# simensov/ml4ca

Hardware: AMD Instinct MI355X
Metric: env-steps/sec at 65536 parallel envs (higher is better)
Workload: dtype f32

## Files before the change

include/dpenv.h:

```cpp
#ifndef DPENV_H
#define DPENV_H

#include <stddef.h>
#include <stdint.h>

#ifdef __cplusplus
extern "C" {
#endif

#define DPENV_ABI_VERSION 6

typedef struct dpenv_s* dpenv_handle;
typedef void* dpenv_stream;

enum {
    DPENV_OK = 0,
    DPENV_EINVAL = -1,
    DPENV_ENODEV = -2,
    DPENV_ENOMEM = -3,
    DPENV_EHIP = -4,
};

enum { DPENV_FULL = 0, DPENV_SIMPLE = 1, DPENV_LIMITED = 2, DPENV_FINAL = 3 };
enum { DPENV_AOS = 0 , DPENV_SOA = 1  };
// ... 80 lines not shown
const char* dpenv_last_error(dpenv_handle h);

int dpenv_set_reset_fraction(dpenv_handle h, float fraction);
int dpenv_set_vessel_class(dpenv_handle h, const int32_t* class_id, dpenv_stream s);

enum { DPENV_VESSEL_KEEP_RANDOMISATION = 1 };
int dpenv_set_vessel_params_ex(dpenv_handle h, const float* params, uint32_t flags, dpenv_stream s);
int dpenv_set_vessel_params(dpenv_handle h, const float* params, dpenv_stream s);
int dpenv_get_vessel_params(dpenv_handle h, float* params_out, dpenv_stream s);
int dpenv_set_vessel_randomisation(dpenv_handle h, const float* nominal, const float* rel_range, dpenv_stream s);
int dpenv_set_current(dpenv_handle h, const float* vc, const float* beta, dpenv_stream s);
int dpenv_set_current_present(dpenv_handle h, const float* vc, const float* beta, dpenv_stream s);
int dpenv_get_current(dpenv_handle h, float* vc_out, float* beta_out, dpenv_stream s);
int dpenv_get_current_mean(dpenv_handle h, float* vc_out, float* beta_out, dpenv_stream s);
int dpenv_set_current_randomisation(dpenv_handle h, const float* vc_nominal, const float* beta_nominal, float vc_range, float beta_range,
                                    dpenv_stream s);

int dpenv_reset(dpenv_handle h, const uint8_t* mask, const float* init, const float* ref, void* obs_out,
                dpenv_stream s);

int dpenv_step(dpenv_handle h, const float* action, const float* new_ref, void* obs_out, float* rew_out,
               uint8_t* done_out, dpenv_stream s);
int dpenv_step_ex(dpenv_handle h, const dpenv_step_io* io, dpenv_stream s);

#define DPENV_MAX_SWITCH 8
typedef struct dpenv_rollout_io {
    uint32_t struct_size;
    int32_t T;
    const float* actions;
    void* obs;
    float* reward;
    uint8_t* done;
    int32_t n_switch;
    int32_t switch_step[DPENV_MAX_SWITCH];
    const float* refs;
} dpenv_rollout_io;
int dpenv_rollout(dpenv_handle h, const dpenv_rollout_io* io, dpenv_stream s);

enum { DPENV_ACT_LEAKY_RELU = 0, DPENV_ACT_TANH = 1 };
typedef struct dpenv_mlp {
    int32_t n_layers;
    int32_t sizes[6];
    const float* W[5];
    const float* b[5];
} dpenv_mlp;
enum { DPENV_POLICY_F16 = 0, DPENV_POLICY_F32 = 1, DPENV_POLICY_F32_ACTOR = 2 };
// ... 204 lines not shown
```

ml4ca_amd/_lib.py:

```python
import ctypes as C
import os

_HERE = os.path.dirname(os.path.abspath(__file__))
LIB_PATH = os.environ.get('DPENV_LIB') or os.path.join(_HERE, 'lib', 'libdpenv.so')

OK, EINVAL, ENODEV, ENOMEM, EHIP = 0, -1, -2, -3, -4
FULL, SIMPLE, LIMITED, FINAL = 0, 1, 2, 3
AOS, SOA = 0, 1
WRAP_REFERENCE, WRAP_RADIANS = 0, 1
F32, BF16 = 0, 1
ACT_LEAKY_RELU, ACT_TANH = 0, 1
IMITATE_NLL, IMITATE_MSE = 0, 1
POLICY_F16, POLICY_F32, POLICY_F32_ACTOR = 0, 1, 2
LAUNCH_AUTO, LAUNCH_ONE_WAVE, LAUNCH_TWO_WAVE = 0, 1, 2
DONE_TERMINAL, DONE_TIMELIMIT, DONE_FAULT = 1, 2, 4
NSTATE, NPARAM, NPARAM_USED, MAX_CLASSES = 15, 32, 32, 64
ABI_VERSION = 6
VESSEL_KEEP_RANDOMISATION = 1

S = dict(N=0, E=1, PSI=2, U=3, V=4, R=5, REF_N=6, REF_E=7, REF_PSI=8,
         PT_BOW=9, PT_PORT=10, PT_STAR=11, A_BOW=12, A_PORT=13, A_STAR=14)
P = dict(M11=0, M22=1, M23=2, M33=3, XU=4, XUU=5, YV=6, YVV=7, YR=8, NV=9, NR=10, NRR=11,
         KF_BOW=12, KF_PORT=13, KF_STAR=14, KR_BOW=15, KR_PORT=16, KR_STAR=17,
         LX_BOW=18, LX_PORT=19, LX_STAR=20, LY_BOW=21, LY_PORT=22, LY_STAR=23, NUV=24, YUR=25,
# ... 87 lines not shown
    'dpenv_abi_version': (C.c_int, []),
    'dpenv_default_config': (C.c_int, [C.POINTER(Config)]),
    'dpenv_default_vessel': (C.c_int, [C.POINTER(C.c_float)]),
    'dpenv_default_vessel_ex': (C.c_int, [C.c_int32, C.POINTER(C.c_float)]),
    'dpenv_act_dim': (C.c_int, [C.POINTER(Config)]),
    'dpenv_obs_dim': (C.c_int, [C.POINTER(Config)]),
    'dpenv_create': (C.c_int, [C.POINTER(Config), C.POINTER(C.c_float), _I32, C.POINTER(_VP)]),
    'dpenv_destroy': (C.c_int, [_VP]),
    'dpenv_last_error': (C.c_char_p, [_VP]),
    'dpenv_set_reset_fraction': (C.c_int, [_VP, _F]),
    'dpenv_set_vessel_class': (C.c_int, [_VP, _VP, _VP]),
    'dpenv_set_vessel_params': (C.c_int, [_VP, _VP, _VP]),
    'dpenv_set_vessel_params_ex': (C.c_int, [_VP, _VP, C.c_uint32, _VP]),
    'dpenv_get_vessel_params': (C.c_int, [_VP, _VP, _VP]),
    'dpenv_set_vessel_randomisation': (C.c_int, [_VP, C.POINTER(C.c_float), C.POINTER(C.c_float), _VP]),
    'dpenv_set_current': (C.c_int, [_VP, _VP, _VP, _VP]),
    'dpenv_set_current_present': (C.c_int, [_VP, _VP, _VP, _VP]),
    'dpenv_get_current': (C.c_int, [_VP, _VP, _VP, _VP]),
    'dpenv_get_current_mean': (C.c_int, [_VP, _VP, _VP, _VP]),
    'dpenv_set_current_randomisation': (C.c_int, [_VP, _VP, _VP, _F, _F, _VP]),
    'dpenv_reset': (C.c_int, [_VP, _VP, _VP, _VP, _VP, _VP]),
    'dpenv_step': (C.c_int, [_VP, _VP, _VP, _VP, _VP, _VP, _VP]),
    'dpenv_step_ex': (C.c_int, [_VP, C.POINTER(StepIO), _VP]),
    'dpenv_rollout': (C.c_int, [_VP, C.POINTER(RolloutIO), _VP]),
    'dpenv_set_policy': (C.c_int, [_VP, C.POINTER(Mlp), C.POINTER(Mlp), C.POINTER(C.c_float), _F]),
    'dpenv_set_policy_ex': (C.c_int, [_VP, C.POINTER(Mlp), C.POINTER(Mlp), C.POINTER(C.c_float), C.c_int32, _F]),
    'dpenv_set_policy_desc': (C.c_int, [_VP, C.POINTER(PolicyDesc), _VP]),
    'dpenv_policy_forward': (C.c_int, [_VP, _VP, _VP, _VP, _I32, _VP]),
    'dpenv_policy_rollout': (C.c_int, [_VP, C.POINTER(PolicyRolloutIO), _VP]),
    'dpenv_get_state': (C.c_int, [_VP, _VP, _VP, _VP]),
    'dpenv_set_state': (C.c_int, [_VP, _VP, _VP, _VP]),
    'dpenv_get_rng_counters': (C.c_int, [_VP, _VP, _VP, _VP]),
    'dpenv_set_rng_counters': (C.c_int, [_VP, _VP, _VP, _VP]),
    'dpenv_get_obs_thrust': (C.c_int, [_VP, _VP, _VP]),
    'dpenv_get_policy_launch': (C.c_int, [_VP, C.POINTER(C.c_int32), C.POINTER(C.c_int32)]),
    'dpenv_get_policy_launch_ex': (C.c_int, [_VP, C.POINTER(C.c_int32)]),
    'dpenv_release_policy_graphs': (C.c_int, [_VP]),
    'dpenv_set_obs_thrust': (C.c_int, [_VP, _VP, _VP]),
    'dpenv_thrust_map': (C.c_int, [C.POINTER(C.c_float), _VP, _VP, _VP, _I32, _VP]),
    'dpenv_gae': (C.c_int, [_VP, _VP, _VP, _VP, _VP, _I32, _I32, _F, _F, _VP, _VP, _VP]),
    'dpenv_gae_workspace_bytes': (C.c_int64, [_I32]),
    'dpenv_gae_stats': (C.c_int, [_VP, _VP, _VP, _VP, _VP, _I32, _I32, _F, _F, _VP, _VP, _VP, _VP, _VP]),
    'dpenv_adv_apply_stats': (C.c_int, [_VP, _I64, _VP, C.c_double, _VP]),
    'dpenv_adv_sum': (C.c_int, [_VP, _I64, _VP, _VP]),
    'dpenv_adv_sumsq': (C.c_int, [_VP, _I64, _VP, _VP, _VP]),
    'dpenv_adv_apply': (C.c_int, [_VP, _I64, _VP, _VP, _VP]),
# ... 78 lines not shown
```

ml4ca_amd/csrc/dpenv_api.hip:

```cpp
#include <cmath>
#include <cstdarg>
#include <cstdio>
#include <cstring>
#include <memory>
#include <new>
#include <string>

#include "dpenv_host.h"

using namespace dpenv;
using namespace dpenv::host;

enum { LOSS_OFF = 0, LOSS_ON = 1, LOSS_UNKNOWN = 2 };

#pragma GCC visibility push(hidden)
struct dpenv_s {
    dpenv_config cfg = {};
    StepArgs args = {};
    int mode = 0;
    int n_classes = 1;
    float* blob = nullptr;
    size_t blob_bytes = 0;
    float* cur_vc = nullptr;
    float* cur_beta = nullptr;
// ... 527 lines not shown
    DeviceGuard dev_guard(h->device);
    if (!io || io->struct_size != sizeof(dpenv_step_io)) return fail(h, DPENV_EINVAL, "dpenv_step_io ABI mismatch");
    if (h->integ_on) return fail(h, DPENV_EINVAL, INTEG_OPEN_LOOP_MSG, "dpenv_step");
    if (h->reff_on) return fail(h, DPENV_EINVAL, REFF_OPEN_LOOP_MSG, "dpenv_step");
    if (!io->action || !io->obs || !io->reward || !io->done)
        return fail(h, DPENV_EINVAL, "action, obs, reward and done buffers are required");
    if (int rc = require_classes(h)) return rc;
    StepArgs a = h->args;
    bind_optional(h, a, (hipStream_t)s);
    a.action = io->action;
    a.new_ref = io->new_ref;
    a.obs = io->obs;
    a.rew = io->reward;
    a.done = io->done;
    a.parts = io->reward_parts;
    a.final_obs = io->final_obs;
    if (!h->has_policy) a.S3 = nullptr;
    const int reset_wave = (!h->cfg.step_one_wave && (int64_t)h->cfg.n_envs <= (int64_t)256 * h->n_cus) ? 1 : 0;
    HIP_TRY(h, dev::launch_step(&a, h->mode, h->cfg.extended_state, vessel_source(h), reset_wave, (hipStream_t)s));
    h->lag_valid = h->has_policy;
    return DPENV_OK;
}

extern "C" int dpenv_step(dpenv_handle h, const float* action, const float* new_ref, void* obs_out, float* rew_out,
                          uint8_t* done_out, dpenv_stream s)
{
    dpenv_step_io io = {};
    io.struct_size = (uint32_t)sizeof io;
    io.action = action; io.new_ref = new_ref; io.obs = obs_out; io.reward = rew_out; io.done = done_out;
    return dpenv_step_ex(h, &io, s);
}

extern "C" int dpenv_rollout(dpenv_handle h, const dpenv_rollout_io* io, dpenv_stream s)
{
    if (!h) return DPENV_EINVAL;
    DeviceGuard dev_guard(h->device);
    if (!io || io->struct_size != sizeof(dpenv_rollout_io)) return fail(h, DPENV_EINVAL, "dpenv_rollout_io ABI mismatch");
    if (h->integ_on) return fail(h, DPENV_EINVAL, INTEG_OPEN_LOOP_MSG, "dpenv_rollout");
    if (h->reff_on) return fail(h, DPENV_EINVAL, REFF_OPEN_LOOP_MSG, "dpenv_rollout");
    if (io->T <= 0 || !io->actions || !io->obs || !io->reward || !io->done)
        return fail(h, DPENV_EINVAL, "T > 0 and action, obs, reward, done blocks are required");
    if (int rc = check_schedule(h, io)) return rc;
    if (int rc = require_classes(h)) return rc;
    StepArgs a = h->args;
    bind_optional(h, a, (hipStream_t)s);
    RolloutArgs ra = {};
// ... 602 lines not shown
```

ml4ca_amd/csrc/dpenv_dev.h:

```cpp
#ifndef DPENV_DEV_H
#define DPENV_DEV_H

#include <hip/hip_runtime.h>
#include <stdint.h>
#include <type_traits>

namespace dpenv {

constexpr int BLOCK = 64;
constexpr int RBLOCK = 64;
constexpr int MAX_SWITCH = 8;
constexpr int CTRL_NPARAM = 32, CTRL_KP = 0, CTRL_KD = 3, CTRL_KI = 6, CTRL_ZB = 9, CTRL_TMAX = 12, CTRL_WEIGHT = 15, CTRL_LX = 20,
              CTRL_LY = 23, CTRL_KF = 26, CTRL_KR_BOW = 29, CTRL_F_EPS = 30;
constexpr int CTRL_TAB_STREAMS = 9;
constexpr int64_t ctrl_tab_float4s(int n) { return ((int64_t)n + 63) / 64 * 64 * CTRL_TAB_STREAMS; }
constexpr int MAX_CLASSES = 64;

enum { MODE_FULL = 0, MODE_SIMPLE = 1, MODE_LIMITED = 2, MODE_FINAL_WRAP = 3, MODE_FINAL_CONT = 4 };
enum { LAYOUT_AOS = 0, LAYOUT_SOA = 1 };
enum { WRAP_REFERENCE = 0, WRAP_RADIANS = 1 };
enum { DONE_TERMINAL = 1u, DONE_TIMELIMIT = 2u, DONE_FAULT = 4u };

enum {
    VD_M11 = 0, VD_M22, VD_M23, VD_INV11, VD_I22, VD_I23, VD_I33,
// ... 283 lines not shown
struct ScoreArgs {
    uint4* state;
    const void* obs;
    const float* act;
    const float* rew;
    const uint8_t* done;
    const float* integ;
    int T, n, obs_stride, act_stride, cut_at_end;
    float dt;
    float norm[3], coeff[3], rps[3];
};

struct LabelArgs {
    const void* obs;
    const uint8_t* done;
    const float* z_in;
    float* z_out;
    float* act;
    int T, n;
};

namespace __attribute__((visibility("hidden"))) dev {
hipError_t launch_step(const StepArgs* a, int mode, int ext, int ves, int reset_wave, hipStream_t s);
hipError_t launch_rollout(const StepArgs* a, const RolloutArgs* ra, int mode, int ext, int ves, int two_wave, hipStream_t s);
hipError_t launch_reset(const StepArgs* a, int mode, int ext, const uint8_t* mask, const float* init, const float* ref, hipStream_t s);
hipError_t launch_get_state(const StepArgs* a, float* st, int32_t* ctr, hipStream_t s);
hipError_t launch_set_state(const StepArgs* a, const float* st, const int32_t* ctr, hipStream_t s);
hipError_t launch_pack_env_vessels(const float* raw, int64_t p_stride, int64_t i_stride, float4* tab, uint32_t* loss_flag, int stride, int n,
                                   hipStream_t s);
hipError_t launch_unpack_env_vessels(const float4* tab, int stride, float* out, int n, hipStream_t s);
hipError_t launch_thrust_map(const VesselDev* vd, const float* n_pct, const float* alpha, float* tau, int n, hipStream_t s);
int64_t gae_workspace_bytes(int n);
hipError_t launch_gae(const float* rew, const float* val, const uint8_t* end, const float* boot, const float* last_val, int T, int n,
                      float gamma, float lam, float* adv, float* ret, double* workspace, double* stats, hipStream_t s);
int64_t score_state_bytes(int n);
int64_t score_summary_workspace_bytes(int n);
hipError_t launch_score(const ScoreArgs* a, int obs_bf16, hipStream_t s);
hipError_t launch_score_read(const void* state, int n, double* out, hipStream_t s);
hipError_t launch_score_summary(const void* state, int n, double* out, double* workspace, hipStream_t s);
hipError_t launch_sum(const float* x, int64_t count, const float* mean, float* out, hipStream_t s);
hipError_t launch_adv_apply(float* x, int64_t count, const float* mean, const float* std, const double* stats, double total_count,
                            hipStream_t s);
hipError_t launch_pack_policy(const PackNet* pi, const PackNet* v, const float* log_std, int adim, int ks, int nent, int nblk, int split,
                              void* frags, float* bias, float* consts, hipStream_t s);
hipError_t launch_policy_forward(const PolicyArgs* pa, int od, int adim, const float* obs, float* mu, float* v, int n, hipStream_t s);
hipError_t launch_policy_forward_x(const PolicyArgs* pa, int od, int adim, const float* obs, float* mu, float* v, int n, hipStream_t s);
// ... 22 lines not shown
```

ml4ca_amd/csrc/dpenv_env_dev.h:

```cpp
#ifndef DPENV_ENV_DEV_H
#define DPENV_ENV_DEV_H
#include <hip/hip_runtime.h>
#include <hip/hip_bf16.h>
#include <stdint.h>

#include "dpenv_dev.h"

namespace dpenv {

constexpr float kPi = 3.14159265358979323846f;

__device__ __forceinline__ void philox4x32_10(uint32_t c0, uint32_t c1, uint32_t c2, uint32_t c3, uint32_t k0,
                                              uint32_t k1, uint32_t out[4])
{
#pragma unroll
    for (int r = 0; r < 10; ++r) {
        const uint64_t p0 = (uint64_t)c0 * 0xD2511F53ull, p1 = (uint64_t)c2 * 0xCD9E8D57ull;
        const uint32_t hi0 = (uint32_t)(p0 >> 32), lo0 = (uint32_t)p0, hi1 = (uint32_t)(p1 >> 32), lo1 = (uint32_t)p1;
        const uint32_t n0 = hi1 ^ c1 ^ k0, n2 = hi0 ^ c3 ^ k1;
        c0 = n0; c1 = lo1; c2 = n2; c3 = lo0;
        k0 += 0x9E3779B9u; k1 += 0xBB67AE85u;
    }
    out[0] = c0; out[1] = c1; out[2] = c2; out[3] = c3;
}
// ... 589 lines not shown
        ang[1] = clipf(w3 * kPi, kPi); ang[2] = clipf(w4 * kPi, kPi);
    } else if (MODE == MODE_FINAL_CONT) {
        if (!DEFER_ANG) { ang[1] = clipf(atan2_lean(act[3], act[4]), kPi); ang[2] = clipf(atan2_lean(act[5], act[6]), kPi); }
    }
}

template <int MODE, bool DEFER_ANG = false>
__device__ __forceinline__ void env_decode(const Vessel& ve, float ang[3], const float* act, Wrench& w, const ThrustLoss* tl = nullptr)
{
    env_decode_cmd<MODE, DEFER_ANG>(ang, act, w.thr);
    if (MODE == MODE_FINAL_CONT) {
        float sc[4];
        const float np2 = fmaf(act[3], act[3], act[4] * act[4]), ns2 = fmaf(act[5], act[5], act[6] * act[6]);
        const float ip = __builtin_amdgcn_rsqf(np2), is = __builtin_amdgcn_rsqf(ns2);
        constexpr float kMinNormal = 1.17549435e-38f;
        sc[0] = (np2 >= kMinNormal) ? act[3] * ip : 0.0f; sc[1] = (np2 >= kMinNormal) ? act[4] * ip : copysignf(1.0f, act[4]);
        sc[2] = (ns2 >= kMinNormal) ? act[5] * is : 0.0f; sc[3] = (ns2 >= kMinNormal) ? act[6] * is : copysignf(1.0f, act[6]);
        thrust_map(ve, w.thr, ang, w.tx, w.ty, w.tn, sc, tl);
    } else {
        thrust_map(ve, w.thr, ang, w.tx, w.ty, w.tn, nullptr, tl);
    }
}

__device__ __forceinline__ void env_plant(const StepArgs& a, const Vessel& ve, float tx, float ty, float tn, bool cur, float vcN,
                                          float vcE, float& N, float& E, float& psi, float& u, float& v, float& r, float sn, float cs)
{
    if (cur) {
        u -= fmaf(cs, vcN, sn * vcE);
        v -= fmaf(cs, vcE, -(sn * vcN));
    }
    const float h = a.h;
    const float hA = h * ve.inv11, h22 = h * ve.i22, h23 = h * ve.i23, h33 = h * ve.i33;
    const float yur = ve.Yur + ve.m11;
    const float nuv = ve.Nuv - ve.m11;
    const int nsub = a.hold_plant ? 0 : a.n_substeps;
    float aN = 0.0f, aE = 0.0f;
#pragma unroll 10
    for (int k = 0; k < nsub; ++k) {
        const float q = fmaf(ve.m22, v, ve.m23 * r);
        float fx = fmaf(-fmaf(ve.Xuu, fabsf(u), ve.Xu), u, tx);
        fx = fmaf(q, r, fx);
        float fy = fmaf(-fmaf(ve.Yvv, fabsf(v), ve.Yv), v, ty);
        fy = fmaf(-fmaf(yur, u, ve.Yr), r, fy);
        float fn = fmaf(-q, u, tn);
        fn = fmaf(-fmaf(nuv, u, ve.Nv), v, fn);
        fn = fmaf(-fmaf(ve.Nrr, fabsf(r), ve.Nr), r, fn);
        u = fmaf(hA, fx, u);
        v = fmaf(h22, fy, fmaf(h23, fn, v));
        r = fmaf(h23, fy, fmaf(h33, fn, r));
        aN = fmaf(-sn, v, fmaf(cs, u, aN));
        aE = fmaf(cs, v, fmaf(sn, u, aE));
        const float d = h * r;
        const float e = -0.5f * d;
        psi += d;
        const float c2 = fmaf(fmaf(e, cs, -sn), d, cs);
        const float s2n = fmaf(fmaf(e, sn, cs), d, sn);
        cs = c2; sn = s2n;
// ... 54 lines not shown
        for (int k = 0; k < 6; ++k) t = t || (fabsf(o[k]) > b[k]);
        d = t ? DONE_TERMINAL : 0u;
    }
    {
        float chk = s.N + s.E + s.psi + s.u + s.v + s.r;
#pragma unroll
        for (int k = 0; k < ModeTraits<MODE>::A; ++k) chk += act[k];
        if (!(fabsf(chk) <= 3.0e38f)) d |= DONE_TERMINAL | DONE_FAULT;
    }
    if (has_ref) { s.refN = nrN; s.refE = nrE; s.refPsi = nrP; }
    s.steps += 1;
    if (a.max_ep_len > 0 && s.steps >= a.max_ep_len) d |= DONE_TIMELIMIT;
    s.pt[0] = thr[0]; s.pt[1] = thr[1]; s.pt[2] = thr[2];
    out.d = d;
}

struct StepRest {
    float thr[3], pt_old[3], ang_prev[3], ang_new[3];
};

template <int MODE, bool EXT, bool DEFER>
__device__ __forceinline__ void env_step_chain(const StepArgs& a, const Vessel& ve, Env& s, const float* act, bool has_ref,
                                               float nrN, float nrE, float nrP, bool cur, float vcN, float vcE, StepOut& out, StepRest& rest,
                                               int il = -1)
{
#pragma unroll
    for (int k = 0; k < 3; ++k) { rest.ang_prev[k] = s.ang[k]; rest.pt_old[k] = s.pt[k]; }
    Wrench w;
    if (il == IL_SHARED || (il >= 0 && thrust_loss_on(a))) {
        ThrustLoss tl;
        if (il == IL_SHARED) {
#pragma unroll
            for (int k = 0; k < 3; ++k) { tl.klf[k] = a.kl[k]; tl.klr[k] = a.kl[3 + k]; }
        } else {
            const float4 q0 = a.env_tab[(int64_t)ENV_GROUPS * a.env_stride + il], q1 = a.env_tab[(int64_t)(ENV_GROUPS + 1) * a.env_stride + il];
            tl.klf[0] = q0.x; tl.klf[1] = q0.y; tl.klf[2] = q0.z; tl.klr[0] = q0.w; tl.klr[1] = q1.x; tl.klr[2] = q1.y;
        }
        tl.u = s.u; tl.v = s.v; tl.r = s.r;
        if (cur) {
            tl.u -= fmaf(s.cs, vcN, s.sn * vcE);
            tl.v -= fmaf(s.cs, vcE, -(s.sn * vcN));
        }
        env_decode<MODE, DEFER>(ve, s.ang, act, w, &tl);
    } else {
        env_decode<MODE, DEFER>(ve, s.ang, act, w);
    }
#pragma unroll
    for (int k = 0; k < 3; ++k) { rest.thr[k] = w.thr[k]; rest.ang_new[k] = s.ang[k]; }
    float N = s.N, E = s.E, psi = s.psi, u = s.u, v = s.v, r = s.r;
    env_plant(a, ve, w.tx, w.ty, w.tn, cur, vcN, vcE, N, E, psi, u, v, r, s.sn, s.cs);
    const bool deg = (a.wrap_mode == WRAP_REFERENCE);
    float* o = out.o;
    bool same;
    float se, ce;
    {
        make_obs(N, E, psi, 0.0f, 0.0f, 0.0f, s.refN, s.refE, s.refPsi, rest.pt_old, deg, o, se, ce, same);
        if (!same) sincos_lean(psi, se, ce);
    }
    env_plant_finish(cur, vcN, vcE, se, ce, u, v);
    o[3] = u; o[4] = v; o[5] = r;
    s.N = N; s.E = E; s.psi = psi; s.u = u; s.v = v; s.r = r;
    s.sn = se; s.cs = ce;
    env_done<MODE>(a, s, act, o, rest.thr, has_ref, nrN, nrE, nrP, out);
}

template <int MODE, bool EXT, bool DEFER>
__device__ __forceinline__ void env_step_finish(const StepArgs& a, Env& s, const float* act, StepRest& rest, bool untouched, StepOut& out)
{
    if (DEFER && MODE == MODE_FINAL_CONT) {
        rest.ang_new[1] = clipf(atan2_lean(act[3], act[4]), kPi);
        rest.ang_new[2] = clipf(atan2_lean(act[5], act[6]), kPi);
        if (untouched) { s.ang[1] = rest.ang_new[1]; s.ang[2] = rest.ang_new[2]; }
    }
// ... 96 lines not shown
```

ml4ca_amd/csrc/dpenv_kernels.hip:

```cpp
#include "dpenv_env_dev.h"

namespace dpenv {

constexpr int RESETW_FIELDS = 18;
constexpr int RESETW_FIELDS_RND = 20;

template <int MODE>
__device__ __forceinline__ void reset_wave(const StepArgs& a, float* lds, int lane, int blk)
{
    const int n = a.n;
    const int i = blk * 64 + lane;
    const int il = i < n ? i : n - 1;
    const uint32_t ep = (uint32_t)a.episode[il];
    const float4 rf = a.RF[il];
    Env s;
    s.refN = rf.x; s.refE = rf.y; s.refPsi = rf.z;
    if (a.new_ref) { s.refN = a.new_ref[il]; s.refE = a.new_ref[(int64_t)n + il]; s.refPsi = a.new_ref[2 * (int64_t)n + il]; }
    ResetDraw d;
    reset_draw<MODE>(a, a.env_id_base + i, ep, d);
    float o[9];
    reset_apply<MODE>(a, s, d, o);
    lds[0 * 64 + lane] = s.N; lds[1 * 64 + lane] = s.E; lds[2 * 64 + lane] = s.psi;
#pragma unroll
    for (int k = 0; k < 9; ++k) lds[(3 + k) * 64 + lane] = o[k];
// ... 70 lines not shown
    lds_order<BLOCK>();
    const __amdgpu_buffer_rsrc_t rObs = buf_rsrc(a.obs, n * (4u * OD));
#pragma unroll
    for (int j = 0; j < OD; ++j) buf_store1(rObs, oobs + j * (4u * BLOCK), lds_io[j * BLOCK + tid]);
    __builtin_amdgcn_sched_barrier(0);
    env_step_finish<MODE, EXT, false>(a, s, act, rest, true, out);
    buf_store1(buf_rsrc(a.rew, n * 4u), o4, out.reward);
}

struct BufDesc {
    const void* base;
    uint32_t bytes;
    uint32_t flags;
};
constexpr uint32_t BUF_FLAGS = 0x00020000;
struct StepFixedArgs {
    VesselDev v0;
    float h, inv_dt;
    int32_t pad;
    BufDesc obs, done, rew, new_ref;
    int32_t terminate, max_ep_len;
};
static_assert(sizeof(StepFixedArgs) == 200 && offsetof(StepFixedArgs, obs) == 128, "StepFixedArgs layout");
constexpr int STEP_FIXED_SUBSTEPS = 20;

__device__ __forceinline__ __amdgpu_buffer_rsrc_t buf_rsrc(const BufDesc& d)
{
    __builtin_assume((reinterpret_cast<uintptr_t>(d.base) >> 48) == 0);
    return __builtin_amdgcn_make_buffer_rsrc(const_cast<void*>(d.base), 0, (int)d.bytes, (int)d.flags);
}
template <typename T> __device__ __forceinline__ void fetch_sgpr(T& x) { asm volatile("" : "+s"(x)); }
__device__ __forceinline__ void fetch_sgpr(BufDesc& d) { fetch_sgpr(d.base); fetch_sgpr(d.bytes); fetch_sgpr(d.flags); }

template <int MODE, bool EXT, bool DEG, bool ENDS, bool REF>
__global__ __launch_bounds__(BLOCK) void step_fixed_kernel(float4* S0, float4* S1, float4* S2, float4* RF, const float* action, int n_,
                                                           const StepFixedArgs fx_)
{
    constexpr int A = ModeTraits<MODE>::A;
    constexpr int OD = EXT ? 9 : 6;
    __shared__ float lds_io[BLOCK * 9];
    const int tid = threadIdx.x;
    const uint32_t n = (uint32_t)n_;
    const uint32_t i = blockIdx.x * BLOCK + tid;
    const uint32_t o16 = i * 16u, o4 = i * 4u;
    const uint32_t oact = (blockIdx.x * (BLOCK * A) + tid) * 4u;
    const uint32_t oobs = (blockIdx.x * (BLOCK * OD) + tid) * 4u;
    const __amdgpu_buffer_rsrc_t rS0 = buf_rsrc(S0, n * 16u), rS1 = buf_rsrc(S1, n * 16u), rS2 = buf_rsrc(S2, n * 16u),
                                 rRF = buf_rsrc(RF, n * 16u), rAct = buf_rsrc(action, n * (4u * A));
    StepFixedArgs fx = fx_;
    StepArgs a;
    a.h = fx.h; a.inv_dt = fx.inv_dt;
    a.n_substeps = STEP_FIXED_SUBSTEPS; a.hold_plant = 0;
    a.wrap_mode = DEG ? WRAP_REFERENCE : WRAP_RADIANS;

    float act[A];
#pragma unroll
// ... 22 lines not shown
#pragma unroll
    for (int j = 0; j < A; ++j) lds_io[j * BLOCK + tid] = act[j];
    lds_order<BLOCK>();
#pragma unroll
    for (int k = 0; k < A; ++k) act[k] = lds_io[tid * A + k];
    const Vessel ve = vessel_from_args(fx.v0);

    StepOut out;
    StepRest rest;
    env_step_chain<MODE, EXT, false>(a, ve, s, act, REF, nrN, nrE, nrP, false, 0.0f, 0.0f, out, rest, IL_NONE);
    buf_store4(rS0, o16, s.N, s.E, s.psi, s.u);
    buf_store4(rS1, o16, s.v, s.r, s.ang[1], s.ang[2]);
    buf_store4(rS2, o16, s.pt[0], s.pt[1], s.pt[2], __int_as_float(s.steps));
    if (REF || MODE == MODE_FULL) buf_store4(rRF, o16, s.refN, s.refE, s.refPsi, s.ang[0]);
    buf_store_u8(buf_rsrc(fx.done), i, (uint8_t)out.d);
    __builtin_amdgcn_sched_barrier(0);
    lds_order<BLOCK>();
#pragma unroll
    for (int k = 0; k < OD; ++k) lds_io[tid * OD + k] = out.o[k];
    lds_order<BLOCK>();
    const __amdgpu_buffer_rsrc_t rObs = buf_rsrc(fx.obs);
#pragma unroll
    for (int j = 0; j < OD; ++j) buf_store1(rObs, oobs + j * (4u * BLOCK), lds_io[j * BLOCK + tid]);
    __builtin_amdgcn_sched_barrier(0);
    env_step_finish<MODE, EXT, false>(a, s, act, rest, true, out);
    buf_store1(buf_rsrc(fx.rew), o4, out.reward);
}

template <int MODE, bool EXT, int VES, bool RESETW = false, bool LEAN = false>
__global__ __launch_bounds__(RESETW ? 2 * BLOCK : BLOCK) void step_kernel(const StepArgs a)
{
    const float4 *pS0 = a.S0, *pS1 = a.S1, *pS2 = a.S2, *pRF = a.RF;
    const float* paction = a.action;
    const int pn = a.n, playout = a.action_layout;
    constexpr int A = ModeTraits<MODE>::A;
    constexpr int OD = EXT ? 9 : 6;
    constexpr bool PER_CLASS = VES == VES_CLASS_LDS;
    constexpr bool RND = VES == VES_ENV_RND;
    constexpr bool ENV_VGPR = VES == VES_ENV_VGPR || RND;
    constexpr int IL = VES == VES_ARGS_LOSS ? IL_SHARED : IL_NONE;
    constexpr bool CURR = RND || VES == VES_ARGS_LOSS;
    __shared__ float lds_io[BLOCK * 9];
    __shared__ float lds_cls[PER_CLASS ? VD_COUNT * MAX_CLASSES : 1];
    __shared__ float4 lds_pe[VES == VES_ENV_LDS ? ENV_GROUPS * 64 : 1];
    __shared__ float lds_rst[RESETW ? (CURR ? RESETW_FIELDS_RND : RESETW_FIELDS) * 64 : 1];
    __shared__ uint32_t lds_fin[RESETW ? 64 : 1];
// ... 883 lines not shown

#include "dpenv_score_dev.h"

}

using namespace dpenv;

static bool vessel_source_ok(const StepArgs& a, int ves)
{
    return !(ves >= VES_ENV_VGPR && ves <= VES_ENV_RND && !a.env_tab) && (ves == VES_ARGS_LOSS) == (a.loss_on == LOSS_SHARED);
}

static bool step_lean_ok(const StepArgs& a, int ves)
{
    return ves == VES_ARGS && !a.auto_reset && !a.final_obs && !a.parts && !a.cur_vc && !a.current_drift && !a.S3 && !a.obs_bf16 &&
           a.obs_layout == LAYOUT_AOS && a.action_layout == LAYOUT_AOS && (int64_t)a.n * 36 < ((int64_t)1 << 31);
}

template <typename F> static hipError_t with_flag(bool on, F&& f)
{
    return on ? f(std::true_type{}) : f(std::false_type{});
}

hipError_t dev::launch_step(const StepArgs* a, int mode, int ext, int ves, int reset_wave, hipStream_t s)
{
    if (!vessel_source_ok(*a, ves)) return hipErrorInvalidValue;
    const dim3 grid((a->n + BLOCK - 1) / BLOCK);
    const bool two = a->auto_reset && reset_wave;
    const bool lean = step_lean_ok(*a, ves);
    return with_mode_ext(mode, ext, [&](auto M, auto E) {
        if (lean && a->n_substeps == STEP_FIXED_SUBSTEPS && !a->hold_plant) {
            StepFixedArgs fx;
            fx.v0 = a->v0;
            fx.h = a->h; fx.inv_dt = a->inv_dt; fx.pad = 0;
            const uint32_t n = (uint32_t)a->n;
            constexpr uint32_t OD = decltype(E)::value ? 9u : 6u;
            fx.obs = {a->obs, n * (4u * OD), BUF_FLAGS};
            fx.done = {a->done, n, BUF_FLAGS};
            fx.rew = {a->rew, n * 4u, BUF_FLAGS};
            fx.new_ref = {a->new_ref, n * 12u, BUF_FLAGS};
            fx.terminate = a->terminate; fx.max_ep_len = a->max_ep_len;
            return with_flag(a->wrap_mode == WRAP_REFERENCE, [&](auto DEG) {
                return with_flag(a->terminate || a->max_ep_len > 0, [&](auto ENDS) { return with_flag(a->new_ref != nullptr, [&](auto REF) {
                    hipLaunchKernelGGL((step_fixed_kernel<M, E, DEG, ENDS, REF>), grid, dim3(BLOCK), 0, s, a->S0, a->S1, a->S2, a->RF, a->action,
                                       a->n, fx);
                    return hipGetLastError();
                }); });
            });
        }
        if (lean) {
            hipLaunchKernelGGL((step_kernel<M, E, VES_ARGS, false, true>), grid, dim3(BLOCK), 0, s, *a);
            return hipGetLastError();
        }
        return with_ves(ves, [&](auto V) {
            if (two) hipLaunchKernelGGL((step_kernel<M, E, V, true>), grid, dim3(2 * BLOCK), 0, s, *a);
            else hipLaunchKernelGGL((step_kernel<M, E, V>), grid, dim3(BLOCK), 0, s, *a);
            return hipGetLastError();
        });
    });
}

hipError_t dev::launch_pack_env_vessels(const float* raw, int64_t p_stride, int64_t i_stride, float4* tab, uint32_t* loss_flag, int stride, int n,
                                        hipStream_t s)
{
    hipLaunchKernelGGL(pack_env_vessels_kernel, dim3((n + BLOCK - 1) / BLOCK), dim3(BLOCK), 0, s, raw, p_stride, i_stride, tab, loss_flag, stride, n);
    return hipGetLastError();
}

hipError_t dev::launch_unpack_env_vessels(const float4* tab, int stride, float* out, int n, hipStream_t s)
{
    hipLaunchKernelGGL(unpack_env_vessels_kernel, dim3((n + BLOCK - 1) / BLOCK), dim3(BLOCK), 0, s, tab, stride, out, n);
    return hipGetLastError();
}
// ... 115 lines not shown
```

ml4ca_amd/env.py:

```python
import ctypes as C
import math
import weakref

import numpy as np

from . import _lib
from .deploy import REFERENCE_FILTER_OMEGA, REFERENCE_FILTER_ZETA
from . import reset_samplers as simtools

_VARIANTS = {'full': _lib.FULL, 'simple': _lib.SIMPLE, 'limited': _lib.LIMITED, 'final': _lib.FINAL}
_NAMES = {'full': 'full', 'simple': 'revoltsimple', 'limited': 'revoltlimited', 'final': 'revoltfinal'}


def variant_constants(variant, cont_ang=False):
    pi = math.pi
    if variant == 'full':
        return dict(num_actions=6, real_action_bounds=[100] * 3 + [pi] * 3,
                    real_ss_bounds=[8.0, 8.0, pi / 2, 1.4, 0.30, 0.52],
                    default_actions={0: 0, 1: 0, 2: 0, 3: 0, 4: 0, 5: 0},
                    valid_action_indices=[0, 1, 2, 3, 4, 5],
                    act_2_act_map={0: 0, 1: 1, 2: 2, 3: 3, 4: 4, 5: 5},
                    act_2_act_map_inv={0: 0, 1: 1, 2: 2, 3: 3, 4: 4, 5: 5})
    if variant == 'simple':
        return dict(num_actions=3, real_action_bounds=[100] * 3,
# ... 14 lines not shown


class Box(object):

    def __init__(self, low, high, dtype=np.float64):
        self.low, self.high, self.shape, self.dtype = low, high, low.shape, dtype

    def sample(self):
        return np.random.uniform(self.low, self.high).astype(self.dtype)


def _torch():
    import torch
    return torch


class BatchedRevoltEnv(object):

    def __init__(self, n_envs, variant='final', extended_state=True, cont_ang=True, device='cuda:0',
                 testing=False, realtime=False, max_ep_len=800, auto_reset=False, terminate=True,
                 wrap_mode='reference', seed=0, env_id_base=0, obs_dtype='float32', current=False,
                 vessel_params=None, layout='aos', reset_fraction=0.8, time_limit=True, hold_plant=False,
                 current_drift=False, current_tau=100.0, current_sigma_v=0.02, current_sigma_beta=5.0 * math.pi / 180.0,
                 n_steps=None, reset_acts=False, step_one_wave=False, per_env_lds=False):
        torch = _torch()
        if not torch.cuda.is_available():
            raise RuntimeError('BatchedRevoltEnv needs a ROCm device: the env.step path is a HIP kernel and has no CPU fallback')
        self.lib = _lib.load()
        self.device = torch.device(device)
        self.variant = variant
        k = variant_constants(variant, cont_ang)
        self.name = _NAMES[variant]
        self.extended_state = bool(extended_state)
        self.cont_ang = bool(cont_ang) and variant == 'final'
        self.testing = bool(testing)
        self.reset_actions = bool(reset_acts)
        self.n_envs = int(n_envs)
        self.num_actions = k['num_actions']
        self.num_states = 9 if extended_state else 6
        self.real_action_bounds = k['real_action_bounds']
        self.real_ss_bounds = k['real_ss_bounds']
        self.default_actions = k['default_actions']
        self.valid_action_indices = k['valid_action_indices']
        self.act_2_act_map = k['act_2_act_map']
        self.act_2_act_map_inv = k['act_2_act_map_inv']
        self.n_steps = 1 if (testing and realtime) else 20
        if n_steps is not None:
            self.n_steps = int(n_steps)
        self.dt = 0.01 * self.n_steps
        self.max_ep_len = int(max_ep_len * 10.0 / self.n_steps)
        self.vel_rew_coeffs = [0.5, 0.5, 1.0]
        self.covar = np.array([[1.0, 0.0], [0.0, 25.0]])
        self.observation_space = Box(-np.ones(self.num_states), np.ones(self.num_states))
        self.action_space = Box(-np.ones(self.num_actions), np.ones(self.num_actions))

        cfg = _lib.default_config()
        cfg.n_envs = self.n_envs
        cfg.device = self.device.index if self.device.index is not None else torch.cuda.current_device()
        cfg.variant = _VARIANTS[variant]
        cfg.extended_state = int(self.extended_state)
        cfg.cont_ang = int(self.cont_ang)
        cfg.n_substeps = self.n_steps
        cfg.substep_dt = 0.01
        cfg.wrap_mode = {'reference': _lib.WRAP_REFERENCE, 'radians': _lib.WRAP_RADIANS}[wrap_mode]
        cfg.terminate = int(bool(terminate))
        cfg.max_ep_len = self.max_ep_len if time_limit else 0
        cfg.auto_reset = int(bool(auto_reset))
        lay = {'aos': _lib.AOS, 'soa': _lib.SOA}[layout]
        cfg.action_layout = lay
        cfg.obs_layout = lay
        self.obs_torch_dtype = {'float32': torch.float32, 'bfloat16': torch.bfloat16}[str(obs_dtype).replace('torch.', '')]
        cfg.obs_dtype = _lib.BF16 if self.obs_torch_dtype == torch.bfloat16 else _lib.F32
        cfg.current_enabled = int(bool(current))
        cfg.seed = int(seed)
        cfg.env_id_base = int(env_id_base)
        cfg.reset_fraction = float(reset_fraction)
        cfg.hold_plant = int(bool(hold_plant))
        cfg.current_drift = int(bool(current_drift))
        cfg.current_tau = float(current_tau)
        cfg.current_sigma_v = float(current_sigma_v)
        cfg.current_sigma_beta = float(current_sigma_beta)
        cfg.reset_acts = int(self.reset_actions)
        cfg.step_one_wave = int(bool(step_one_wave))
        cfg.per_env_lds = int(bool(per_env_lds))
        self.cfg = cfg
        self.layout = layout
# ... 100 lines not shown
        f32, chk = self._f32, self._chk
        chk(action, self._ashape, f32, 'action')
        if out is None:
            obs, rew, done = self._next_obs(), self._rew, self._done
        else:
            obs, rew, done = out
            chk(obs, self._oshape, self.obs_torch_dtype, 'out[0]')
            chk(rew, self._n1, f32, 'out[1]')
            chk(done, self._n1, self._u8, 'out[2]')
        io = self._io
        io.action = action.data_ptr()
        io.new_ref = chk(new_ref, self._r3, f32, 'new_ref').data_ptr() if new_ref is not None else None
        io.obs = obs.data_ptr()
        io.reward = rew.data_ptr()
        io.done = done.data_ptr()
        io.reward_parts = chk(reward_parts, self._p4, f32, 'reward_parts').data_ptr() if reward_parts is not None else None
        io.final_obs = chk(final_obs, self._oshape, self.obs_torch_dtype, 'final_obs').data_ptr() if final_obs is not None else None
        rc = self._step_ex(self._h, self._io_ref, self._stream())
        if rc:
            self._refuse_open_loop('step')
            _lib.check(rc, self._h)
        return obs, rew, done, {'None': 0}

    def _refuse_open_loop(self, what):
        if self.integral_action is not None:
            raise ValueError('%s(): the integral action is on (set_integral_action) and this launch\'s observations would lack I; fly the closed '
                             'loop (policy.policy_rollout), compose step() with deploy.BatchedBodyFrameIntegrator after set_integral_action(None), '
                             'or turn it off' % what)
        if self.reference_filter is not None:
            raise ValueError('%s(): the reference filter is on (set_reference_filter) and would not see this launch; fly the closed loop '
                             '(policy.policy_rollout), compose step() with deploy.BatchedReferenceFilter (its position as new_ref) after '
                             'set_reference_filter(None), or turn it off' % what)

    def rollout(self, actions, switch_steps=(), refs=None, out=None):
        torch = _torch()
        self._refuse_open_loop('rollout')
        T = int(actions.shape[0])
        n = self.n_envs
        self._chk(actions, (T,) + self.action_shape, torch.float32, 'actions')
        k = len(switch_steps)
        if k > 8:
            raise ValueError('at most 8 setpoint switches per rollout launch')
        if k:
            self._chk(refs, (k, 3, n), torch.float32, 'refs')
        if out is None:
            obs = torch.empty((T,) + self.obs_shape, dtype=self.obs_torch_dtype, device=self.device)
# ... 461 lines not shown
```

Measured before the change: 14.79 billion.

## Add wide fixed-step kernel with vectorized block-staged action/obs I/O

Adds a step_fixed_wide_kernel used when n is a multiple of 4 and the action/obs pointers are 16-byte aligned. It loads actions and stores observations as per-block float4 rows staged through LDS, instead of per-element strided scalar accesses. It also precomputes the plant constants on the host and passes them as kernel arguments, avoiding per-thread recomputation. The kernel argument block grows, and the new path adds extra LDS barriers plus more code to maintain. It also exposes a dpenv_step_form query and a substep_dt option.

```diff
diff --git a/include/dpenv.h b/include/dpenv.h
--- a/include/dpenv.h
+++ b/include/dpenv.h
@@ -126,6 +126,8 @@
 int dpenv_step(dpenv_handle h, const float* action, const float* new_ref, void* obs_out, float* rew_out,
                uint8_t* done_out, dpenv_stream s);
 int dpenv_step_ex(dpenv_handle h, const dpenv_step_io* io, dpenv_stream s);
+enum { DPENV_STEP_FORM_GENERAL = 0, DPENV_STEP_FORM_LEAN = 1, DPENV_STEP_FORM_FIXED = 2, DPENV_STEP_FORM_FIXED_WIDE = 3 };
+int dpenv_step_form(dpenv_handle h, const dpenv_step_io* io);
 
 #define DPENV_MAX_SWITCH 8
 typedef struct dpenv_rollout_io {
diff --git a/ml4ca_amd/_lib.py b/ml4ca_amd/_lib.py
--- a/ml4ca_amd/_lib.py
+++ b/ml4ca_amd/_lib.py
@@ -133,6 +133,7 @@
     'dpenv_reset': (C.c_int, [_VP, _VP, _VP, _VP, _VP, _VP]),
     'dpenv_step': (C.c_int, [_VP, _VP, _VP, _VP, _VP, _VP, _VP]),
     'dpenv_step_ex': (C.c_int, [_VP, C.POINTER(StepIO), _VP]),
+    'dpenv_step_form': (C.c_int, [_VP, C.POINTER(StepIO)]),
     'dpenv_rollout': (C.c_int, [_VP, C.POINTER(RolloutIO), _VP]),
     'dpenv_set_policy': (C.c_int, [_VP, C.POINTER(Mlp), C.POINTER(Mlp), C.POINTER(C.c_float), _F]),
     'dpenv_set_policy_ex': (C.c_int, [_VP, C.POINTER(Mlp), C.POINTER(Mlp), C.POINTER(C.c_float), C.c_int32, _F]),
diff --git a/ml4ca_amd/csrc/dpenv_api.hip b/ml4ca_amd/csrc/dpenv_api.hip
--- a/ml4ca_amd/csrc/dpenv_api.hip
+++ b/ml4ca_amd/csrc/dpenv_api.hip
@@ -573,6 +573,26 @@
     return DPENV_OK;
 }
 
+extern "C" int dpenv_step_form(dpenv_handle h, const dpenv_step_io* io)
+{
+    if (!h) return DPENV_EINVAL;
+    if (!io || io->struct_size != sizeof(dpenv_step_io)) return fail(h, DPENV_EINVAL, "dpenv_step_io ABI mismatch");
+    DeviceGuard dev_guard(h->device);
+    StepArgs a = h->args;
+    bind_optional(h, a, nullptr);
+    a.action = io->action;
+    a.new_ref = io->new_ref;
+    a.obs = io->obs;
+    a.rew = io->reward;
+    a.done = io->done;
+    a.parts = io->reward_parts;
+    a.final_obs = io->final_obs;
+    if (!h->has_policy) a.S3 = nullptr;
+    static_assert(dev::STEP_FORM_GENERAL == DPENV_STEP_FORM_GENERAL && dev::STEP_FORM_LEAN == DPENV_STEP_FORM_LEAN &&
+                  dev::STEP_FORM_FIXED == DPENV_STEP_FORM_FIXED && dev::STEP_FORM_FIXED_WIDE == DPENV_STEP_FORM_FIXED_WIDE, "dpenv.h step forms");
+    return dev::step_form(&a, vessel_source(h));
+}
+
 extern "C" int dpenv_step(dpenv_handle h, const float* action, const float* new_ref, void* obs_out, float* rew_out,
                           uint8_t* done_out, dpenv_stream s)
 {
diff --git a/ml4ca_amd/csrc/dpenv_dev.h b/ml4ca_amd/csrc/dpenv_dev.h
--- a/ml4ca_amd/csrc/dpenv_dev.h
+++ b/ml4ca_amd/csrc/dpenv_dev.h
@@ -329,6 +329,8 @@
 
 namespace __attribute__((visibility("hidden"))) dev {
 hipError_t launch_step(const StepArgs* a, int mode, int ext, int ves, int reset_wave, hipStream_t s);
+enum { STEP_FORM_GENERAL = 0, STEP_FORM_LEAN = 1, STEP_FORM_FIXED = 2, STEP_FORM_FIXED_WIDE = 3 };
+int step_form(const StepArgs* a, int ves);
 hipError_t launch_rollout(const StepArgs* a, const RolloutArgs* ra, int mode, int ext, int ves, int two_wave, hipStream_t s);
 hipError_t launch_reset(const StepArgs* a, int mode, int ext, const uint8_t* mask, const float* init, const float* ref, hipStream_t s);
 hipError_t launch_get_state(const StepArgs* a, float* st, int32_t* ctr, hipStream_t s);
diff --git a/ml4ca_amd/csrc/dpenv_env_dev.h b/ml4ca_amd/csrc/dpenv_env_dev.h
--- a/ml4ca_amd/csrc/dpenv_env_dev.h
+++ b/ml4ca_amd/csrc/dpenv_env_dev.h
@@ -635,17 +635,23 @@
     }
 }
 
+struct PlantConsts {
+    float hA, h22, h23, h33, yur, nuv;
+};
+
 __device__ __forceinline__ void env_plant(const StepArgs& a, const Vessel& ve, float tx, float ty, float tn, bool cur, float vcN,
-                                          float vcE, float& N, float& E, float& psi, float& u, float& v, float& r, float sn, float cs)
+                                          float vcE, float& N, float& E, float& psi, float& u, float& v, float& r, float sn, float cs,
+                                          const PlantConsts* pre = nullptr)
 {
     if (cur) {
         u -= fmaf(cs, vcN, sn * vcE);
         v -= fmaf(cs, vcE, -(sn * vcN));
     }
     const float h = a.h;
-    const float hA = h * ve.inv11, h22 = h * ve.i22, h23 = h * ve.i23, h33 = h * ve.i33;
-    const float yur = ve.Yur + ve.m11;
-    const float nuv = ve.Nuv - ve.m11;
+    const float hA = pre ? pre->hA : h * ve.inv11, h22 = pre ? pre->h22 : h * ve.i22, h23 = pre ? pre->h23 : h * ve.i23,
+                h33 = pre ? pre->h33 : h * ve.i33;
+    const float yur = pre ? pre->yur : ve.Yur + ve.m11;
+    const float nuv = pre ? pre->nuv : ve.Nuv - ve.m11;
     const int nsub = a.hold_plant ? 0 : a.n_substeps;
     float aN = 0.0f, aE = 0.0f;
 #pragma unroll 10
@@ -746,7 +752,7 @@
 template <int MODE, bool EXT, bool DEFER>
 __device__ __forceinline__ void env_step_chain(const StepArgs& a, const Vessel& ve, Env& s, const float* act, bool has_ref,
                                                float nrN, float nrE, float nrP, bool cur, float vcN, float vcE, StepOut& out, StepRest& rest,
-                                               int il = -1)
+                                               int il = -1, const PlantConsts* pre = nullptr)
 {
 #pragma unroll
     for (int k = 0; k < 3; ++k) { rest.ang_prev[k] = s.ang[k]; rest.pt_old[k] = s.pt[k]; }
@@ -772,7 +778,7 @@
 #pragma unroll
     for (int k = 0; k < 3; ++k) { rest.thr[k] = w.thr[k]; rest.ang_new[k] = s.ang[k]; }
     float N = s.N, E = s.E, psi = s.psi, u = s.u, v = s.v, r = s.r;
-    env_plant(a, ve, w.tx, w.ty, w.tn, cur, vcN, vcE, N, E, psi, u, v, r, s.sn, s.cs);
+    env_plant(a, ve, w.tx, w.ty, w.tn, cur, vcN, vcE, N, E, psi, u, v, r, s.sn, s.cs, pre);
     const bool deg = (a.wrap_mode == WRAP_REFERENCE);
     float* o = out.o;
     bool same;
diff --git a/ml4ca_amd/csrc/dpenv_kernels.hip b/ml4ca_amd/csrc/dpenv_kernels.hip
--- a/ml4ca_amd/csrc/dpenv_kernels.hip
+++ b/ml4ca_amd/csrc/dpenv_kernels.hip
@@ -116,6 +116,22 @@
     int32_t terminate, max_ep_len;
 };
 static_assert(sizeof(StepFixedArgs) == 200 && offsetof(StepFixedArgs, obs) == 128, "StepFixedArgs layout");
+struct BufWords {
+    uint32_t lo, hi, bytes, flags;
+};
+struct alignas(8) StepFixedWideArgs {
+    int32_t lead[4];
+    VesselDev v0;
+    float h, inv_dt;
+    float pad;
+    PlantConsts pc;
+    BufWords obs, done, rew;
+    int32_t terminate, max_ep_len;
+    BufWords new_ref;
+};
+static_assert(offsetof(StepFixedWideArgs, v0) == 16 && offsetof(StepFixedWideArgs, pc) == 144 && offsetof(StepFixedWideArgs, obs) == 168 &&
+              offsetof(StepFixedWideArgs, rew) == 200 && offsetof(StepFixedWideArgs, new_ref) == 224 && sizeof(StepFixedWideArgs) == 240,
+              "StepFixedWideArgs layout: 64-byte pieces from byte 16");
 constexpr int STEP_FIXED_SUBSTEPS = 20;
 
 __device__ __forceinline__ __amdgpu_buffer_rsrc_t buf_rsrc(const BufDesc& d)
@@ -125,7 +141,19 @@
 }
 template <typename T> __device__ __forceinline__ void fetch_sgpr(T& x) { asm volatile("" : "+s"(x)); }
 __device__ __forceinline__ void fetch_sgpr(BufDesc& d) { fetch_sgpr(d.base); fetch_sgpr(d.bytes); fetch_sgpr(d.flags); }
-
+__device__ __forceinline__ void fetch_sgpr(BufWords& d) { fetch_sgpr(d.lo); fetch_sgpr(d.hi); fetch_sgpr(d.bytes); fetch_sgpr(d.flags); }
+__device__ __forceinline__ __amdgpu_buffer_rsrc_t buf_rsrc(const BufWords& d)
+{
+    __builtin_assume((d.hi >> 16) == 0);
+    return __builtin_amdgcn_make_buffer_rsrc(reinterpret_cast<void*>((uint64_t)d.hi << 32 | d.lo), 0, (int)d.bytes, (int)d.flags);
+}
+
+template <int ROW> __device__ __forceinline__ __amdgpu_buffer_rsrc_t wide_block_rsrc(const void* base, uint32_t bytes)
+{
+    const uint32_t off = blockIdx.x * (BLOCK * ROW * 4u);
+    const uint32_t left = bytes - off;
+    return buf_rsrc(static_cast<const char*>(base) + off, left < BLOCK * ROW * 4u ? left : BLOCK * ROW * 4u);
+}
 template <int MODE, bool EXT, bool DEG, bool ENDS, bool REF>
 __global__ __launch_bounds__(BLOCK) void step_fixed_kernel(float4* S0, float4* S1, float4* S2, float4* RF, const float* action, int n_,
                                                            const StepFixedArgs fx_)
@@ -194,6 +222,93 @@
     const __amdgpu_buffer_rsrc_t rObs = buf_rsrc(fx.obs);
 #pragma unroll
     for (int j = 0; j < OD; ++j) buf_store1(rObs, oobs + j * (4u * BLOCK), lds_io[j * BLOCK + tid]);
+    __builtin_amdgcn_sched_barrier(0);
+    env_step_finish<MODE, EXT, false>(a, s, act, rest, true, out);
+    buf_store1(buf_rsrc(fx.rew), o4, out.reward);
+}
+
+template <int MODE, bool EXT, bool DEG, bool ENDS, bool REF>
+__global__ __launch_bounds__(BLOCK) void step_fixed_wide_kernel(float4* S0, float4* S1, float4* S2, float4* RF, const float* action, int n_,
+                                                                const StepFixedWideArgs fx_)
+{
+    constexpr int A = ModeTraits<MODE>::A;
+    constexpr int OD = EXT ? 9 : 6;
+    constexpr int AW = (A + 3) / 4, OW = (OD + 3) / 4;
+    __shared__ __attribute__((aligned(16))) float lds_io[BLOCK * 4 * OW];
+    static_assert(AW <= OW, "the action pieces fit the image");
+    const int tid = threadIdx.x;
+    const uint32_t n = (uint32_t)n_;
+    const uint32_t i = blockIdx.x * BLOCK + tid;
+    const uint32_t o16 = i * 16u, o4 = i * 4u;
+    const uint32_t ow = tid * 16u;
+    const __amdgpu_buffer_rsrc_t rS0 = buf_rsrc(S0, n * 16u), rS1 = buf_rsrc(S1, n * 16u), rS2 = buf_rsrc(S2, n * 16u),
+                                 rRF = buf_rsrc(RF, n * 16u), rAct = wide_block_rsrc<A>(action, n * (4u * A));
+    StepFixedWideArgs fx = fx_;
+    StepArgs a;
+    a.h = fx.h; a.inv_dt = fx.inv_dt;
+    a.n_substeps = STEP_FIXED_SUBSTEPS; a.hold_plant = 0;
+    a.wrap_mode = DEG ? WRAP_REFERENCE : WRAP_RADIANS;
+
+    float4 actw[AW];
+#pragma unroll
+    for (int j = 0; j < AW; ++j) actw[j] = buf_load4(rAct, ow + j * 1024u);
+    __builtin_amdgcn_sched_barrier(0);
+    Env s;
+    {
+        const float4 s0 = buf_load4(rS0, o16), s1 = buf_load4(rS1, o16), s2 = buf_load4(rS2, o16), rf = buf_load4(rRF, o16);
+        s.N = s0.x; s.E = s0.y; s.psi = s0.z; s.u = s0.w; s.v = s1.x; s.r = s1.y;
+        s.ang[0] = rf.w; s.ang[1] = s1.z; s.ang[2] = s1.w;
+        s.pt[0] = s2.x; s.pt[1] = s2.y; s.pt[2] = s2.z; s.steps = __float_as_int(s2.w);
+        s.refN = rf.x; s.refE = rf.y; s.refPsi = rf.z;
+    }
+    float nrN = 0.0f, nrE = 0.0f, nrP = 0.0f;
+    if (REF) {
+        const __amdgpu_buffer_rsrc_t rNR = buf_rsrc(fx.new_ref);
+        nrN = buf_load1(rNR, o4); nrE = buf_load1(rNR, o4 + n * 4u); nrP = buf_load1(rNR, o4 + n * 8u);
+    }
+#pragma unroll
+    for (int k = 0; k < VD_COUNT; ++k) fetch_sgpr(fx.v0.p[k]);
+    fetch_sgpr(fx.h); fetch_sgpr(fx.inv_dt); fetch_sgpr(fx.pad);
+    fetch_sgpr(fx.pc.hA); fetch_sgpr(fx.pc.h22); fetch_sgpr(fx.pc.h23); fetch_sgpr(fx.pc.h33); fetch_sgpr(fx.pc.yur); fetch_sgpr(fx.pc.nuv);
+    fetch_sgpr(fx.done); fetch_sgpr(fx.rew);
+    if (ENDS) { fetch_sgpr(fx.terminate); fetch_sgpr(fx.max_ep_len); }
+    a.terminate = ENDS ? fx.terminate : 0; a.max_ep_len = ENDS ? fx.max_ep_len : 0;
+    BufWords ob;
+    {
+        const uint32_t off = blockIdx.x * (BLOCK * OD * 4u), left = fx.obs.bytes - off;
+        const uint64_t base = ((uint64_t)fx.obs.hi << 32 | fx.obs.lo) + off;
+        ob = {(uint32_t)base, (uint32_t)(base >> 32), left < BLOCK * OD * 4u ? left : BLOCK * OD * 4u, fx.obs.flags};
+        fetch_sgpr(ob);
+    }
+    __builtin_amdgcn_sched_barrier(0);
+    sincos_lean(s.psi, s.sn, s.cs);
+#pragma unroll
+    for (int j = 0; j < AW; ++j) reinterpret_cast<float4*>(lds_io)[j * BLOCK + tid] = actw[j];
+    lds_order<BLOCK>();
+    float act[A];
+#pragma unroll
+    for (int k = 0; k < A; ++k) act[k] = lds_io[tid * A + k];
+    const Vessel ve = vessel_from_args(fx.v0);
+
+    StepOut out;
+    StepRest rest;
+    env_step_chain<MODE, EXT, false>(a, ve, s, act, REF, nrN, nrE, nrP, false, 0.0f, 0.0f, out, rest, IL_NONE, &fx.pc);
+    buf_store4(rS0, o16, s.N, s.E, s.psi, s.u);
+    buf_store4(rS1, o16, s.v, s.r, s.ang[1], s.ang[2]);
+    buf_store4(rS2, o16, s.pt[0], s.pt[1], s.pt[2], __int_as_float(s.steps));
+    if (REF || MODE == MODE_FULL) buf_store4(rRF, o16, s.refN, s.refE, s.refPsi, s.ang[0]);
+    buf_store_u8(buf_rsrc(fx.done), i, (uint8_t)out.d);
+    __builtin_amdgcn_sched_barrier(0);
+    lds_order<BLOCK>();
+#pragma unroll
+    for (int k = 0; k < OD; ++k) lds_io[tid * OD + k] = out.o[k];
+    lds_order<BLOCK>();
+    const __amdgpu_buffer_rsrc_t rObs = buf_rsrc(ob);
+#pragma unroll
+    for (int j = 0; j < OW; ++j) {
+        const float4 q = reinterpret_cast<const float4*>(lds_io)[j * BLOCK + tid];
+        buf_store4(rObs, ow + j * 1024u, q.x, q.y, q.z, q.w);
+    }
     __builtin_amdgcn_sched_barrier(0);
     env_step_finish<MODE, EXT, false>(a, s, act, rest, true, out);
     buf_store1(buf_rsrc(fx.rew), o4, out.reward);
@@ -1123,33 +1238,74 @@
     return on ? f(std::true_type{}) : f(std::false_type{});
 }
 
+static StepFixedArgs step_fixed_args(const StepArgs& a, uint32_t od)
+{
+    StepFixedArgs fx;
+    const uint32_t n = (uint32_t)a.n;
+    fx.v0 = a.v0;
+    fx.h = a.h; fx.inv_dt = a.inv_dt; fx.pad = 0;
+    fx.obs = {a.obs, n * (4u * od), BUF_FLAGS};
+    fx.done = {a.done, n, BUF_FLAGS};
+    fx.rew = {a.rew, n * 4u, BUF_FLAGS};
+    fx.new_ref = {a.new_ref, n * 12u, BUF_FLAGS};
+    fx.terminate = a.terminate; fx.max_ep_len = a.max_ep_len;
+    return fx;
+}
+
+static StepFixedWideArgs step_fixed_wide_args(const StepArgs& a, uint32_t od)
+{
+    StepFixedWideArgs fx = {};
+    const uint32_t n = (uint32_t)a.n;
+    fx.v0 = a.v0;
+    fx.h = a.h; fx.inv_dt = a.inv_dt;
+    const float* v = a.v0.p;
+    fx.pc.hA = a.h * v[VD_INV11]; fx.pc.h22 = a.h * v[VD_I22]; fx.pc.h23 = a.h * v[VD_I23]; fx.pc.h33 = a.h * v[VD_I33];
+    fx.pc.yur = v[VD_YUR] + v[VD_M11]; fx.pc.nuv = v[VD_NUV] - v[VD_M11];
+    const auto words = [](const void* p, uint32_t bytes) {
+        const uint64_t b = reinterpret_cast<uintptr_t>(p);
+        return BufWords{(uint32_t)b, (uint32_t)(b >> 32), bytes, BUF_FLAGS};
+    };
+    fx.obs = words(a.obs, n * (4u * od));
+    fx.done = words(a.done, n);
+    fx.rew = words(a.rew, n * 4u);
+    fx.new_ref = words(a.new_ref, n * 12u);
+    fx.terminate = a.terminate; fx.max_ep_len = a.max_ep_len;
+    return fx;
+}
+
+int dev::step_form(const StepArgs* a, int ves)
+{
+    if (!step_lean_ok(*a, ves)) return STEP_FORM_GENERAL;
+    if (a->n_substeps != STEP_FIXED_SUBSTEPS || a->hold_plant) return STEP_FORM_LEAN;
+    const uintptr_t rows = reinterpret_cast<uintptr_t>(a->action) | reinterpret_cast<uintptr_t>(a->obs);
+    return (a->n % 4 == 0 && (rows & 15u) == 0) ? STEP_FORM_FIXED_WIDE : STEP_FORM_FIXED;
+}
+
 hipError_t dev::launch_step(const StepArgs* a, int mode, int ext, int ves, int reset_wave, hipStream_t s)
 {
     if (!vessel_source_ok(*a, ves)) return hipErrorInvalidValue;
     const dim3 grid((a->n + BLOCK - 1) / BLOCK);
     const bool two = a->auto_reset && reset_wave;
-    const bool lean = step_lean_ok(*a, ves);
+    const int form = step_form(a, ves);
     return with_mode_ext(mode, ext, [&](auto M, auto E) {
-        if (lean && a->n_substeps == STEP_FIXED_SUBSTEPS && !a->hold_plant) {
-            StepFixedArgs fx;
-            fx.v0 = a->v0;
-            fx.h = a->h; fx.inv_dt = a->inv_dt; fx.pad = 0;
-            const uint32_t n = (uint32_t)a->n;
+        if (form == STEP_FORM_FIXED || form == STEP_FORM_FIXED_WIDE) {
             constexpr uint32_t OD = decltype(E)::value ? 9u : 6u;
-            fx.obs = {a->obs, n * (4u * OD), BUF_FLAGS};
-            fx.done = {a->done, n, BUF_FLAGS};
-            fx.rew = {a->rew, n * 4u, BUF_FLAGS};
-            fx.new_ref = {a->new_ref, n * 12u, BUF_FLAGS};
-            fx.terminate = a->terminate; fx.max_ep_len = a->max_ep_len;
+            const bool wide = form == STEP_FORM_FIXED_WIDE;
+            const StepFixedArgs fx = wide ? StepFixedArgs{} : step_fixed_args(*a, OD);
+            const StepFixedWideArgs fw = wide ? step_fixed_wide_args(*a, OD) : StepFixedWideArgs{};
             return with_flag(a->wrap_mode == WRAP_REFERENCE, [&](auto DEG) {
                 return with_flag(a->terminate || a->max_ep_len > 0, [&](auto ENDS) { return with_flag(a->new_ref != nullptr, [&](auto REF) {
-                    hipLaunchKernelGGL((step_fixed_kernel<M, E, DEG, ENDS, REF>), grid, dim3(BLOCK), 0, s, a->S0, a->S1, a->S2, a->RF, a->action,
-                                       a->n, fx);
+                    if (wide)
+                        hipLaunchKernelGGL((step_fixed_wide_kernel<M, E, DEG, ENDS, REF>), grid, dim3(BLOCK), 0, s, a->S0, a->S1, a->S2, a->RF,
+                                           a->action, a->n, fw);
+                    else
+                        hipLaunchKernelGGL((step_fixed_kernel<M, E, DEG, ENDS, REF>), grid, dim3(BLOCK), 0, s, a->S0, a->S1, a->S2, a->RF, a->action,
+                                           a->n, fx);
                     return hipGetLastError();
                 }); });
             });
         }
-        if (lean) {
+        if (form == STEP_FORM_LEAN) {
             hipLaunchKernelGGL((step_kernel<M, E, VES_ARGS, false, true>), grid, dim3(BLOCK), 0, s, *a);
             return hipGetLastError();
         }
diff --git a/ml4ca_amd/env.py b/ml4ca_amd/env.py
--- a/ml4ca_amd/env.py
+++ b/ml4ca_amd/env.py
@@ -60,7 +60,7 @@
                  wrap_mode='reference', seed=0, env_id_base=0, obs_dtype='float32', current=False,
                  vessel_params=None, layout='aos', reset_fraction=0.8, time_limit=True, hold_plant=False,
                  current_drift=False, current_tau=100.0, current_sigma_v=0.02, current_sigma_beta=5.0 * math.pi / 180.0,
-                 n_steps=None, reset_acts=False, step_one_wave=False, per_env_lds=False):
+                 n_steps=None, reset_acts=False, step_one_wave=False, per_env_lds=False, substep_dt=0.01):
         torch = _torch()
         if not torch.cuda.is_available():
             raise RuntimeError('BatchedRevoltEnv needs a ROCm device: the env.step path is a HIP kernel and has no CPU fallback')
@@ -85,7 +85,7 @@
         self.n_steps = 1 if (testing and realtime) else 20
         if n_steps is not None:
             self.n_steps = int(n_steps)
-        self.dt = 0.01 * self.n_steps
+        self.dt = float(substep_dt) * self.n_steps
         self.max_ep_len = int(max_ep_len * 10.0 / self.n_steps)
         self.vel_rew_coeffs = [0.5, 0.5, 1.0]
         self.covar = np.array([[1.0, 0.0], [0.0, 25.0]])
@@ -99,7 +99,7 @@
         cfg.extended_state = int(self.extended_state)
         cfg.cont_ang = int(self.cont_ang)
         cfg.n_substeps = self.n_steps
-        cfg.substep_dt = 0.01
+        cfg.substep_dt = float(substep_dt)
         cfg.wrap_mode = {'reference': _lib.WRAP_REFERENCE, 'radians': _lib.WRAP_RADIANS}[wrap_mode]
         cfg.terminate = int(bool(terminate))
         cfg.max_ep_len = self.max_ep_len if time_limit else 0
@@ -246,6 +246,32 @@
             _lib.check(rc, self._h)
         return obs, rew, done, {'None': 0}
 
+    STEP_FORMS = ('general', 'lean', 'fixed', 'fixed_wide')
+
+    def step_form(self, action, new_ref=None, out=None, reward_parts=None, final_obs=None):
+        f32, chk = self._f32, self._chk
+        chk(action, self._ashape, f32, 'action')
+        if out is None:
+            obs, rew, done = self._obs[self._flip ^ 1], self._rew, self._done
+        else:
+            obs, rew, done = out
+            chk(obs, self._oshape, self.obs_torch_dtype, 'out[0]')
+            chk(rew, self._n1, f32, 'out[1]')
+            chk(done, self._n1, self._u8, 'out[2]')
+        io = _lib.StepIO()
+        io.struct_size = C.sizeof(_lib.StepIO)
+        io.action = action.data_ptr()
+        io.new_ref = chk(new_ref, self._r3, f32, 'new_ref').data_ptr() if new_ref is not None else None
+        io.obs = obs.data_ptr()
+        io.reward = rew.data_ptr()
+        io.done = done.data_ptr()
+        io.reward_parts = chk(reward_parts, self._p4, f32, 'reward_parts').data_ptr() if reward_parts is not None else None
+        io.final_obs = chk(final_obs, self._oshape, self.obs_torch_dtype, 'final_obs').data_ptr() if final_obs is not None else None
+        rc = self.lib.dpenv_step_form(self._h, C.byref(io))
+        if rc < 0:
+            _lib.check(rc, self._h)
+        return self.STEP_FORMS[rc]
+
     def _refuse_open_loop(self, what):
         if self.integral_action is not None:
             raise ValueError('%s(): the integral action is on (set_integral_action) and this launch\'s observations would lack I; fly the closed '
```

Measured after the change: 14.96 billion, median of 2. No clear change (+1.1%).
